# AshutoshNirkhe/KubernetesClusterCapacity

Hardware: AMD Instinct MI355X
Metric: node×spec fit evals/sec at 1M nodes × 4K specs; % of HBM roofline (higher is better)
Workload: dtype int64; 1 GPU; C4: 1000000 nodes x 20000000 pods x 4096 specs; reduce + fit prepare + fit + finalize; nodes=1000000, pods=20000000, containers_rank0=39602467, nodes_rank0=1000000, pods_rank0=19801877, pods_per_node=poisson, mean 20, specs=4096, parallelism=node-sharded x1

## Files before the change

### include/kcc.h

```cpp
#ifndef KCC_H
#define KCC_H

#include <stdint.h>

#ifdef __cplusplus
extern "C" {
#endif

#define KCC_ABI_VERSION 2

enum {
  KCC_OK = 0,
  KCC_EINVAL = -1,
  KCC_ENOMEM = -2,
  KCC_EHIP = -3,
  KCC_ENODEV = -4,
  KCC_ERCCL = -5,
  KCC_EFAULT = -6
};

enum {
  KCC_SPEC_OK = 0,
  KCC_SPEC_DIVZERO = 1,
  KCC_SPEC_FAULT = 2
// ... 93 lines not shown
int kcc_p2p_open(kcc_ctx* ctx, int rank, const uint8_t* handles );
int kcc_exchange_finalize_async(kcc_ctx* ctx, int64_t n_specs, const int64_t* d_partial,
                                int64_t* d_totals, int32_t* d_spec_err, void* stream);
int kcc_p2p_faults(kcc_ctx* ctx, int64_t* faults);

int kcc_profile_enable(kcc_ctx* ctx, int on);
int kcc_profile_read(kcc_ctx* ctx, double* reduce_ms, int64_t* reduce_launches, double* fit_ms,
                     int64_t* fit_launches);

int kcc_reduce_faults(kcc_ctx* ctx, int64_t* faults);
int kcc_clear_faults(kcc_ctx* ctx);

int kcc_set_fit_dense(kcc_ctx* ctx, int dense);
int kcc_set_clamp_in_fit(kcc_ctx* ctx, int mode);
int kcc_clamp_in_fit_used(kcc_ctx* ctx, int* used);
int kcc_fit_stream_rows(kcc_ctx* ctx, int64_t* streamed);

double kcc_last_slow_fraction(const kcc_ctx* ctx);

int kcc_fit_slow_pairs(kcc_ctx* ctx, int64_t* slow_pairs, int64_t* pairs);

enum {
  KCC_PARSE_OK = 1,
  KCC_PARSE_ERR = 0,
  KCC_PARSE_UNSUPPORTED = -1,
  KCC_PARSE_BADOFF = -2
};
int kcc_parse_cpu_millis(kcc_ctx* ctx, int64_t n, const char* bytes, int64_t n_bytes,
                         const int64_t* offsets, uint64_t* out, int8_t* status);
int kcc_parse_bytes(kcc_ctx* ctx, int64_t n, const char* bytes, int64_t n_bytes,
// ... 71 lines not shown
```

### kubernetesclustercapacity_amd/_lib.py

```python
from __future__ import annotations

import ctypes as C
import os
import re

_HERE = os.path.dirname(os.path.abspath(__file__))
LIB_PATH = os.path.join(_HERE, "libkcc.so")
HEADER_PATH = os.path.join(os.path.dirname(_HERE), "include", "kcc.h")

KCC_OK = 0
KCC_EINVAL = -1
KCC_ENOMEM = -2
KCC_EHIP = -3
KCC_ENODEV = -4
KCC_ERCCL = -5
KCC_EFAULT = -6
ERROR_NAMES = {
    KCC_EINVAL: "KCC_EINVAL", KCC_ENOMEM: "KCC_ENOMEM", KCC_EHIP: "KCC_EHIP",
    KCC_ENODEV: "KCC_ENODEV", KCC_ERCCL: "KCC_ERCCL", KCC_EFAULT: "KCC_EFAULT",
}
KCC_SPEC_OK = 0
KCC_SPEC_DIVZERO = 1
KCC_SPEC_FAULT = 2

# ... 12 lines not shown
    "kcc_reduce_requests_async": (_int, [_vp, _i64, _i64] + [_vp] * 10),
    "kcc_fit": (_int, [_vp, _i64] + [_vp] * 6 + [_i64] + [_vp] * 4),
    "kcc_capacity": (_int, [_vp, _i64, _i64] + [_vp] * 7 + [_i64] + [_vp] * 4),
    "kcc_fit_partial_async": (_int, [_vp, _i64] + [_vp] * 6 + [_i64] + [_vp] * 4),
    "kcc_fit_prepare_async": (_int, [_vp, _i64] + [_vp] * 6 + [_i64] + [_vp] * 4),
    "kcc_fit_run_async": (_int, [_vp, _i64, _i64, _vp, _vp]),
    "kcc_fit_finalize_async": (_int, [_vp, _i64, _vp, _vp, _vp, _vp]),
    "kcc_fit_async": (_int, [_vp, _i64] + [_vp] * 6 + [_i64] + [_vp] * 5),
    "kcc_capacity_partial_async": (_int, [_vp, _i64, _i64] + [_vp] * 10 + [_i64] + [_vp] * 3
                                   + [_int, _vp]),
    "kcc_capacity_async": (_int, [_vp, _i64, _i64] + [_vp] * 10 + [_i64] + [_vp] * 5),
    "kcc_set_node_shards": (_int, [_vp, _int]),
    "kcc_set_fit_dense": (_int, [_vp, _int]),
    "kcc_set_clamp_in_fit": (_int, [_vp, _int]),
    "kcc_clamp_in_fit_used": (_int, [_vp, C.POINTER(C.c_int)]),
    "kcc_fit_stream_rows": (_int, [_vp, C.POINTER(_i64)]),
    "kcc_reduce_faults": (_int, [_vp, C.POINTER(_i64)]),
    "kcc_clear_faults": (_int, [_vp]),
    "kcc_comm_unique_id": (_int, [_vp]),
    "kcc_comm_init": (_int, [_vp, _vp, _int, _int]),
    "kcc_allreduce_partial_async": (_int, [_vp, _i64, _vp, _vp]),
    "kcc_p2p_export": (_int, [_vp, _int, _i64, _vp]),
    "kcc_p2p_open": (_int, [_vp, _int, _vp]),
    "kcc_exchange_finalize_async": (_int, [_vp, _i64, _vp, _vp, _vp, _vp]),
    "kcc_p2p_faults": (_int, [_vp, C.POINTER(_i64)]),
    "kcc_profile_enable": (_int, [_vp, _int]),
    "kcc_profile_read": (_int, [_vp] + [C.POINTER(_dbl), C.POINTER(_i64)] * 2),
    "kcc_last_slow_fraction": (_dbl, [_vp]),
    "kcc_fit_slow_pairs": (_int, [_vp, C.POINTER(_i64), C.POINTER(_i64)]),
    "kcc_parse_cpu_millis": (_int, [_vp, _i64, _vp, _i64, _vp, _vp, _vp]),
# ... 61 lines not shown
```

### kubernetesclustercapacity_amd/csrc/kcc_abi.cpp

```cpp
#include "kcc.h"

#include <hip/hip_runtime.h>
#include <rccl/rccl.h>

#include <cstdio>
#include <cstdlib>
#include <cstring>
#include <string>
#include <vector>

#include "kcc_internal.h"

namespace {

struct DevBuf {
  void* p = nullptr;
  size_t bytes = 0;
};

hipError_t ensure(DevBuf& b, size_t bytes) {
  if (bytes == 0) bytes = 16;
  if (b.bytes >= bytes) return hipSuccess;
  if (b.p) (void)hipFree(b.p);
  b.p = nullptr;
// ... 38 lines not shown
  DevBuf fast_a, fast_b, slow, slow_list, srec, sperm, counters;
  DevBuf red_tail;
  DevBuf faults;
  DevBuf rank_arrive;
  DevBuf fit_q;
  bool fitq_dirty = true;
  DevBuf c_rank, c_bcnt, c_cs, c_ms, c_mrc, c_crm, c_dperm;
  DevBuf c_C, c_H2, c_H3, c_Crow, c_rec, c_dir;
  bool clamp_dirty = true;
  int64_t last_pairs = 0;
  int64_t c_stride = 0;
  int64_t h_stride = 0;
  int64_t d_stride = 0;
  bool fit_dense = false;
  int clamp_in_fit = -1;
  bool last_nc = false;
  DevBuf fast_cl;
  int stream_chunks = 0;
  int64_t prep_nodes = -1, prep_specs = -1;
  DevBuf ptr, cpu, mem, cpul, meml, used_cpu, used_mem, lim_cpu, lim_mem;
  DevBuf alloc_cpu, alloc_mem, alloc_pods, pod_count, spec_cpu, spec_mem, partial, totals, err;
  DevBuf p_bytes, p_off, p_out, p_st;
  DevBuf k_key;
  DevBuf g_group;
  DevBuf g_count, g_cursor, g_total, g_rec, g_rg, g_acc;
  DevBuf kb_counts, kb_tot, kb_sr, kb_sv;
  DevBuf kb_part, kb_arrive;
  DevBuf kb_esc_n, kb_esc_row, kb_esc_cpu, kb_esc_mem;
  DevBuf q_ptr, q_iptr, q_icpu, q_imem, q_rst, q_ocpu, q_omem, q_pcpu, q_pmem;
  DevBuf p2p_mbox, p2p_arrive;
// ... 428 lines not shown
  dv.stream_chunks = k;
  dv.prep_nodes = -1;
  dv.prep_specs = -1;
  hipStream_t rs = k > 1 ? dv.side : s;
  if (k > 1) {
    KCC_HIP(ctx, hipEventRecord(dv.ev_fork, s));
    KCC_HIP(ctx, hipStreamWaitEvent(dv.side, dv.ev_fork, 0));
  }
  const bool fuse_place = n_specs > 0;
  const bool fuse_rank = k == 1 && fuse_place && n_nodes > 0 && n_cont > 0;
  const bool nc = fuse_rank && n_specs <= kcc::CLAMP_LDS_SPECS && !dv.fit_dense &&
                  (dv.clamp_in_fit == 1 ||
                   (dv.clamp_in_fit < 0 && kcc::clamp_in_fit_auto(n_nodes, n_specs)));
  int32_t* const fast_cl = nc ? as<int32_t>(dv.fast_cl) : nullptr;
  dv.last_nc = nc;
  kcc::RankArgs ra = kcc::rank_args(n_specs, spec_cpu, spec_mem, clamp_of(dv),
                                    as<unsigned long long>(dv.counters),
                                    as<uint32_t>(dv.rank_arrive), nc);
  kcc::PlaceArgs pa = place_args(dv, n_specs, spec_cpu, spec_mem, partial);
  pa.no_ranks = nc ? 1 : 0;
  kcc::NpArgs np{};
  if (nc) {
    ra.done_flag = as<uint32_t>(dv.np_sync);
    np.n_place = (int32_t)((n_specs + 255) / 256);
    np.n_rows = (int32_t)((n_nodes + kcc::NP_ROWS_PER_WG - 1) / kcc::NP_ROWS_PER_WG);
    np.sync = as<uint32_t>(dv.np_sync);
    np.pa = pa;
    np.n = n_nodes;
    np.alloc_cpu = alloc_cpu;
    np.alloc_mem = alloc_mem;
// ... 48 lines not shown
    KCC_HIP(ctx, kcc::launch_node_prep(n, alloc_cpu + lo[c], alloc_mem + lo[c], alloc_pods + lo[c],
                                       pod_count + lo[c], used_cpu + lo[c], used_mem + lo[c],
                                       as<kcc::FitGroupA>(dv.fast_a) + lo[c] / kcc::FIT_GROUP,
                                       as<kcc::FitGroup>(dv.fast_b) + lo[c] / kcc::FIT_GROUP,
                                       as<kcc::SlowNode>(dv.slow) + lo[c],
                                       as<int64_t>(dv.slow_list) + lo[c], n_specs, clamp_of(dv),
                                       as<unsigned long long>(dv.counters),
                                       c, lo[c], n_nodes, s, dv.fit_dense,
                                       place_here ? &pa : nullptr));
    if (n == 0) continue;
    ProfPair pp{};
    if (dv.prof_on) {
      KCC_HIP(ctx, prof_event(dv, &pp.a));
      KCC_HIP(ctx, prof_event(dv, &pp.b));
    }
    KCC_HIP(ctx, kcc::launch_fit(n, as<kcc::FitGroupA>(dv.fast_a) + lo[c] / kcc::FIT_GROUP,
                                 as<kcc::FitGroup>(dv.fast_b) + lo[c] / kcc::FIT_GROUP,
                                 as<kcc::SlowNode>(dv.slow) + lo[c],
                                 as<int64_t>(dv.slow_list) + lo[c], n_specs, spec_prep_of(dv),
                                 partial, as<unsigned long long>(dv.counters),
                                 as<uint32_t>(dv.fit_q), c, n_nodes, s,
                                 as<const unsigned long long>(dv.faults), fast_cl,
                                 dv.prof_on ? pp.a : nullptr, dv.prof_on ? pp.b : nullptr));
    if (dv.prof_on) {
      pp.kind = 1;
      dv.prof_pending.push_back(pp);
    }
  }
  if (n_specs > 0 && nc) {
    dv.clamp_dirty = false;
    if (totals) return fit_finalize_dev(ctx, dv, n_specs, partial, totals, spec_err, s);
    return KCC_OK;
  }
  if (n_specs > 0) {
    if (n_nodes > 0)
      KCC_HIP(ctx, kcc::launch_clamp_apply(n_specs, n_nodes, clamp_of(dv),
                                           as<unsigned long long>(dv.counters), partial, s,
                                           fuse_fin ? &fin : nullptr));
    dv.clamp_dirty = false;
    if (totals && !fuse_fin)
      return fit_finalize_dev(ctx, dv, n_specs, partial, totals, spec_err, s);
  }
  return KCC_OK;
}
// ... 549 lines not shown

int kcc_clamp_in_fit_used(kcc_ctx* ctx, int* used) {
  if (!ctx || !used) return KCC_EINVAL;
  *used = 0;
  for (const Dev& dv : ctx->devs) *used |= dv.last_nc ? 1 : 0;
  return KCC_OK;
}

int kcc_set_clamp_in_fit(kcc_ctx* ctx, int mode) {
  if (!ctx) return KCC_EINVAL;
  if (mode < -1 || mode > 1) return fail(ctx, KCC_EINVAL, "mode: -1 (by size), 0 or 1");
  for (Dev& dv : ctx->devs) dv.clamp_in_fit = mode;
  return KCC_OK;
}

int kcc_fit_stream_rows(kcc_ctx* ctx, int64_t* streamed) {
  if (!ctx || !streamed) return ctx ? fail(ctx, KCC_EINVAL, "NULL output") : KCC_EINVAL;
  if (ctx->host_stream_rows >= 0) {
    *streamed = ctx->host_stream_rows;
    return KCC_OK;
  }
  Dev& dv = ctx->devs[0];
  KCC_HIP(ctx, hipSetDevice(dv.device));
  KCC_HIP(ctx, hipDeviceSynchronize());
  unsigned long long c[kcc::CNT_N] = {};
  if (dv.counters.p)
    KCC_HIP(ctx, hipMemcpy(c, dv.counters.p, sizeof(c), hipMemcpyDeviceToHost));
  int64_t t = 0;
  for (int k = 0; k < dv.stream_chunks && k < kcc::FIT_MAX_CHUNKS; ++k) t += (int64_t)c[kcc::CNT_STREAM + k];
  *streamed = t;
// ... 759 lines not shown
```

### kubernetesclustercapacity_amd/csrc/kcc_internal.h

```cpp
#pragma once
#include <hip/hip_runtime.h>
#include <stdint.h>

#if !defined(KCC_VARIANT_BUILD) &&                                                       \
    (defined(KCC_DIAG_RED_NOSTORE) || defined(KCC_DIAG_RED_LOADONLY) ||                  \
     defined(KCC_TIMELINE) || defined(KCC_DIAG_RED_GIVEUP) || defined(KCC_DIAG_P2P_GIVEUP) || \
     defined(KCC_DIAG_INLIB_COMM) || defined(KCC_DIAG_GA_NOATOM) ||                     \
     defined(KCC_DIAG_NP_NOSC1))
#error "a diagnostic KCC_* knob in a release build: use `make variant` (KCC_VARIANT_BUILD)"
#endif

namespace kcc {

struct RankArgs;
struct NpArgs;

constexpr int RED_PREFETCH = 1;
constexpr int RED_IPL = 8;
constexpr int RED_TILE = 64 * RED_IPL;
constexpr int RED_WAVES_PER_BLOCK = 4;
constexpr int64_t RED_MAX_NODES = (int64_t)1 << 28;
constexpr int RED_TAIL_WORDS = 8;
constexpr int RED_TAIL_TAG = 7;
constexpr uint64_t RED_TAG_READY = 1;
// ... 207 lines not shown
                            unsigned long long* counters, int chunk, int64_t row0,
                            int64_t call_nodes, hipStream_t s, bool dense = false,
                            const PlaceArgs* place = nullptr);
constexpr int64_t CLAMP_IN_FIT_PAIRS = 1100000000LL;
inline bool clamp_in_fit_auto(int64_t n_nodes, int64_t n_specs) {
  return n_specs <= CLAMP_LDS_SPECS && n_nodes * n_specs <= CLAMP_IN_FIT_PAIRS;
}

hipError_t launch_fit(int64_t n_nodes, const FitGroupA* fast_a, const FitGroup* fast_b,
                      const SlowNode* slow,
                      const int64_t* slow_list, int64_t n_specs, SpecPrep sp, int64_t* partial,
                      unsigned long long* counters, uint32_t* queue, int chunk,
                      int64_t grid_nodes, hipStream_t s, const unsigned long long* faults,
                      const int32_t* fast_cl = nullptr, hipEvent_t ev_start = nullptr,
                      hipEvent_t ev_stop = nullptr);
constexpr int64_t FIT_QSUBS_MAX = 32;
inline int64_t fit_queue_words(int64_t S) { return (S + 255) / 256 * FIT_QSUBS_MAX * 16; }

hipError_t launch_fit_finalize(int64_t n_specs, const int64_t* partial,
                               const int32_t* perm, int64_t* totals, int32_t* spec_err,
                               const unsigned long long* faults, hipStream_t s);
hipError_t launch_partial_add(int64_t n, int64_t* dst, const int64_t* src, hipStream_t s);

constexpr int P2P_MAX_RANKS = 8;
__host__ __device__ inline size_t p2p_flag_words(int W) { return (size_t)2 * W * 8; }
inline size_t p2p_mbox_bytes(int W, int64_t smax) {
  return 8 * (p2p_flag_words(W) + (size_t)2 * W * 2 * (size_t)smax);
}
struct P2PArgs {
  int64_t S, smax;
// ... 105 lines not shown
```

### kubernetesclustercapacity_amd/csrc/kcc_kernels.hip

```cpp

#include <hip/hip_ext.h>
#include <hip/hip_runtime.h>
#include <stdint.h>

#include <atomic>

#include "kcc_internal.h"

namespace kcc {

namespace {

#ifdef KCC_TIMELINE
__device__ uint64_t kcc_tl[8192][8];
#define KCC_TL(slot, k) \
  do { if (threadIdx.x == 0) kcc_tl[(slot)][(k)] = __builtin_amdgcn_s_memrealtime(); } while (0)
#define KCC_TLV(slot, k, v) \
  do { if (threadIdx.x == 0) kcc_tl[(slot)][(k)] = (v); } while (0)
#else
#define KCC_TL(slot, k) do { } while (0)
#define KCC_TLV(slot, k, v) do { } while (0)
#endif

typedef __attribute__((address_space(3))) unsigned long long lds_ull;
// ... 1449 lines not shown
  rec.rc = normal ? recip_up_f64(c) : 0.0;
  rec.rm = normal ? recip_up_f64((uint64_t)m) : 0.0;
  rec.rcf = cls == SPEC_A ? recip_up_f32(c) : 0.0f;
  rec.cls = cls;
  rec.pad = 0;
  sp.rec[pos] = rec;
  sp.perm[pos] = (int32_t)i;
  partial[i] = 0;
  partial[S + i] = device_faulted(pa.faults) ? (int64_t)SPEC_FAULT_MARK : 0;
  if (!normal || pa.no_ranks) return;
  cw.dperm[x] = (int32_t)pos;
}


constexpr int CP_THREADS = 1024;
constexpr int CP_WAVES = CP_THREADS / 64;
constexpr int64_t C_FULL_CELLS = 4624;
constexpr int H_CELLS = 65 * 64;
__host__ __device__ inline bool clamp_c_full(int64_t T) { return (T + 2) * (T + 2) <= C_FULL_CELLS; }

constexpr int CP_PW = 4096;
constexpr int64_t CP_SPLIT = 4;
constexpr int CP_RB = 8;
__device__ __forceinline__ void clamp_consume_bin(const ClampWork& cw, int64_t bin, uint64_t* tab,
                                                  uint32_t* w_lo, uint32_t* w_off, uint64_t* scratch,
                                                  uint32_t h, uint32_t G) {
  constexpr int PPT = CP_PW / CP_THREADS;
  const int tid = threadIdx.x, lane = tid & 63, wv = tid >> 6;
  uint32_t* wsum = reinterpret_cast<uint32_t*>(scratch);
  for (int64_t p0 = 0; p0 < cw.n_pass; p0 += CP_PW) {
    const int np = (int)(cw.n_pass - p0 < CP_PW ? cw.n_pass - p0 : CP_PW);
    uint32_t lo[PPT], cnt[PPT];
#pragma unroll
    for (int u = 0; u < PPT; ++u) {
      const int p = tid * PPT + u;
      lo[u] = 0;
      cnt[u] = 0;
      if (p < np) {
        const uint32_t* d = cw.dir + (p0 + p) * cw.d_stride + bin;
        lo[u] = d[0];
        cnt[u] = d[1];
      }
    }
    uint32_t ts = 0;
#pragma unroll
    for (int u = 0; u < PPT; ++u) {
      cnt[u] -= lo[u];
      ts += cnt[u];
    }
    uint32_t inc = ts;
#pragma unroll
    for (int d = 1; d < 64; d <<= 1) {
      const uint32_t t = __shfl_up(inc, d, 64);
      if (lane >= d) inc += t;
    }
    if (lane == 63) wsum[wv] = inc;
    __syncthreads();
    uint32_t before = 0, total = 0;
#pragma unroll
    for (int w2 = 0; w2 < CP_WAVES; ++w2) {
      const uint32_t t = wsum[w2];
      before += w2 < wv ? t : 0u;
      total += t;
    }
    uint32_t run = before + inc - ts;
#pragma unroll
    for (int u = 0; u < PPT; ++u) {
      const int p = tid * PPT + u;
      w_lo[p] = lo[u];
      w_off[p] = run;
      run += cnt[u];
    }
    if (tid == 0) w_off[CP_PW] = total;
    __syncthreads();
    int top = 1;
    while (2 * top <= np) top *= 2;
    auto search = [&](uint32_t j) {
      int p = 0;
      for (int st = top; st >= 1; st >>= 1)
        if (w_off[p + st] <= j) p += st;
      return p;
    };
    const uint32_t s0 = (uint32_t)((uint64_t)total * h / G), s1 = (uint32_t)((uint64_t)total * (h + 1) / G);
    const uint32_t per_w = (s1 - s0 + CP_WAVES * 64 - 1) / (CP_WAVES * 64) * 64;
    const uint32_t J0 = s0 + (uint32_t)wv * per_w;
    const uint32_t J1 = J0 + per_w < s1 ? J0 + per_w : s1;
    int p = J0 + lane < J1 ? search(J0 + lane) : 0;
    uint32_t nxt = w_off[p + 1], gb = w_lo[p] - w_off[p];
    const uint64_t* rec0 = cw.rec + p0 * cw.pass_recs;
    auto load_batch = [&](uint64_t (&rv)[CP_RB], uint32_t jb) {
#pragma unroll
      for (int u = 0; u < CP_RB; ++u) {
        const uint32_t j = jb + (uint32_t)(64 * u + lane);
        rv[u] = 0;
        if (j < J1) {
          if (j >= nxt) {
            p = w_off[p + 2] <= j ? search(j) : p + 1;
            nxt = w_off[p + 1];
            gb = w_lo[p] - w_off[p];
          }
          rv[u] = rec0[(int64_t)p * cw.pass_recs + (uint32_t)(j + gb)];
        }
      }
    };
    auto add_batch = [&](const uint64_t (&rv)[CP_RB], uint32_t jb) {
#pragma unroll
      for (int u = 0; u < CP_RB; ++u)
        if (jb + (uint32_t)(64 * u + lane) < J1)
          atomicAdd(reinterpret_cast<unsigned long long*>(&tab[(uint32_t)rv[u]]),
                    (unsigned long long)(int64_t)(int32_t)(rv[u] >> 32));
    };
    const uint32_t step = 64u * CP_RB;
    uint64_t ra[CP_RB], rb[CP_RB];
    load_batch(ra, J0);
    for (uint32_t jb = J0; jb < J1; jb += 2 * step) {
      load_batch(rb, jb + step);
      add_batch(ra, jb);
      load_batch(ra, jb + 2 * step);
      add_batch(rb, jb + step);
    }
    __syncthreads();
  }
}

__device__ __forceinline__ void clamp_apply_bin(const ClampWork& cw, int64_t S,
                                                int64_t* __restrict__ partial, int64_t nN,
                                                int64_t u, uint32_t G, uint32_t h) {
  __shared__ uint64_t tab[H_CELLS];
  __shared__ uint64_t ctot[CP_WAVES][64];
  __shared__ uint64_t colsum[128];
  __shared__ uint32_t pos_s[64];
  __shared__ uint32_t cp_lo[CP_PW];
  __shared__ uint32_t cp_off[CP_PW + 1];
  const int64_t T = (nN + 63) / 64, W = T + 2;
  KCC_TL(1024 + blockIdx.x % 1024, 0);
  const int tid = threadIdx.x, lane = tid & 63, wv = tid >> 6;
  const bool x_side = u < T;
  const int64_t g = x_side ? u : u - T;
  const bool full = clamp_c_full(T);
  const int64_t q = 64 * g + lane;
  uint32_t other = 0xffffffffu;
  if (wv == 0 || wv == CP_WAVES - 1) other = (x_side ? cw.mr_c : cw.cr_m)[q];
  if (tid < 128) colsum[tid] = 0;
  const bool binned = clamp_binned(S);
  int64_t* H = (x_side ? cw.H2 : cw.H3) + g * H_CELLS;
  constexpr int PER = (H_CELLS + CP_THREADS - 1) / CP_THREADS;
  uint64_t v[PER];
#pragma unroll
  for (int k = 0; k < PER; ++k) {
    const int e = tid + CP_THREADS * k;
    v[k] = 0;
    if (!binned) {
#pragma unroll
      for (int c = 0; c < H2_COPIES; ++c) v[k] += e < H_CELLS ? (uint64_t)H[c * cw.h_stride + e] : 0ull;
    }
  }
  constexpr int CPER = (int)((C_FULL_CELLS + CP_THREADS - 1) / CP_THREADS);
  uint64_t cv[CPER];
  const int64_t c0 = (g + 1) * W, c1 = W * W;
  const bool do_c = x_side && full && h == 0;
#pragma unroll
  for (int k = 0; k < CPER; ++k) {
    const int64_t e = c0 + tid + CP_THREADS * k;
    cv[k] = 0;
    if (do_c && e < c1) {
#pragma unroll
      for (int c = 0; c < C_COPIES; ++c) cv[k] += (uint64_t)cw.C[c * cw.c_stride + e];
    }
  }
#pragma unroll
  for (int k = 0; k < PER; ++k) {
    const int e = tid + CP_THREADS * k;
    if (e < H_CELLS) {
      tab[e] = v[k];
      if (!binned) {
#pragma unroll
        for (int c = 0; c < H2_COPIES; ++c) H[c * cw.h_stride + e] = 0;
      }
    }
  }
  __syncthreads();
  KCC_TL(1024 + blockIdx.x % 1024, 1);
  if (binned) clamp_consume_bin(cw, x_side ? g : T + g, tab, cp_lo, cp_off, &ctot[0][0], h, G);
  KCC_TL(1024 + blockIdx.x % 1024, 2);
  if (do_c) {
#pragma unroll
    for (int k = 0; k < CPER; ++k) {
      const int64_t e = c0 + tid + CP_THREADS * k;
      if (e < c1 && cv[k]) atomicAdd(reinterpret_cast<unsigned long long*>(&colsum[e % W]), cv[k]);
    }
  }
  int32_t p = 0x7fffffff;
  if (wv == 0 && q < nN) p = cw.dperm[x_side ? q : (int64_t)other];
  for (int k = wv; k < 65; k += CP_WAVES) {
    const uint64_t sr = wave_incl_scan_u64(tab[k * 64 + 63 - lane]);
    tab[k * 64 + 63 - lane] = sr;
  }
  if (wv == CP_WAVES - 1) {
    uint32_t pos = 0;
    for (int l = 0; l < 64; ++l) pos += (uint32_t)__builtin_amdgcn_readlane((int)other, l) < other ? 1u : 0u;
    pos_s[lane] = pos;
  }
  __syncthreads();
  constexpr int KCH = (65 + CP_WAVES - 1) / CP_WAVES;
  const int k0 = wv * KCH, k1 = k0 + KCH < 65 ? k0 + KCH : 65;
  {
    const uint32_t posl = pos_s[lane];
    uint64_t part = 0;
    for (int k = k0; k < k1; ++k)
      part += (lane < 63 && (uint32_t)k > posl) ? tab[k * 64 + lane + 1] : 0ull;
    ctot[wv][lane] = part;
  }
  __syncthreads();
  if (wv != 0) return;
  KCC_TL(1024 + blockIdx.x % 1024, 3);
  uint64_t csuf = 0;
  if (do_c) {
    uint64_t carry = 0;
    for (int ch = 1; ch >= 0; --ch) {
      const int col = ch * 64 + 63 - lane;
      uint64_t sv = col < W ? colsum[col] : 0ull;
      sv = wave_incl_scan_u64(sv) + carry;
      carry = readlane_u64(sv, 63);
      if (col < W) colsum[col] = sv;
    }
    const uint32_t gy1 = other == 0xffffffffu ? 0xffffffffu : (other >> 6) + 1;
    csuf = gy1 < W ? colsum[gy1] : 0ull;
  }
  if (q >= nN) return;
  uint64_t d = csuf;
#pragma unroll
  for (int w2 = 0; w2 < CP_WAVES; ++w2) d += ctot[w2][lane];
  if (x_side && !full && h == 0) {
    const int64_t gy = other >> 6;
    uint64_t part[8] = {};
    for (int64_t G = g + 1; G <= T + 1; G += 8) {
#pragma unroll
      for (int r = 0; r < 8; ++r)
        part[r] += G + r <= T + 1 ? (uint64_t)cw.Crow[(G + r) * W + gy + 1] : 0ull;
    }
#pragma unroll
    for (int r = 0; r < 8; ++r) d += part[r];
  }
  if (d && p < clamp_n_pure(nN, S)) atomic_add_u64(reinterpret_cast<uint64_t*>(&partial[p]), 0ull - d);
  KCC_TL(1024 + blockIdx.x % 1024, 4);
}

__device__ void fused_finalize(const FinArgs& fin, int64_t S, const int64_t* partial,
// ... 28 lines not shown
      fin.totals[dst[k]] = e[k] != 0 || fk ? 0 : t[k];
      fin.spec_err[dst[k]] = fk ? SPEC_ERR_FAULT : e[k] != 0 ? SPEC_ERR_DIV0 : 0;
    }
  }
}

__global__ __launch_bounds__(CP_THREADS) void clamp_apply_kernel(ClampWork cw,
                                                                 const unsigned long long* __restrict__ counters,
                                                                 int64_t S, int64_t* __restrict__ partial,
                                                                 FinArgs fin) {
  const int64_t nN = clamp_n_normal(counters);
  const int64_t T = (nN + 63) / 64;
  const int64_t Tm = (S + 63) / 64;
  const uint32_t G = gridDim.x / (uint32_t)(2 * Tm), h = blockIdx.x / (uint32_t)(2 * Tm);
  const int64_t u = blockIdx.x % (uint32_t)(2 * Tm);
  if (u < 2 * T) clamp_apply_bin(cw, S, partial, nN, u, G, h);
  if (fin.totals) fused_finalize(fin, S, partial, fin.arrive, gridDim.x, 0, S);
}

__global__ __launch_bounds__(256) void clamp_crows_kernel(ClampWork cw,
                                                          const unsigned long long* __restrict__ counters) {
  const int64_t nN = clamp_n_normal(counters);
  const int64_t T = (nN + 63) / 64, W = T + 2;
  const int64_t G = (int64_t)blockIdx.x * 4 + (threadIdx.x >> 6);
  const int lane = threadIdx.x & 63;
  if (nN == 0 || clamp_c_full(T) || G >= W) return;
  uint64_t carry = 0;
  for (int64_t ch = (W + 63) / 64 - 1; ch >= 0; --ch) {
    const int64_t gy = ch * 64 + 63 - lane;
    uint64_t v = 0;
#pragma unroll
// ... 350 lines not shown
  }
  KCC_TL(2048 + b % 4096, 3);
}

template <bool CL>
__global__ __launch_bounds__(256) KCC_FIT_ATTR void fit_kernel(
    int64_t n_nodes, uint32_t* __restrict__ queue, const FitGroupA* __restrict__ fast_a,
    const FitGroup* __restrict__ fast_b, const SlowNode* __restrict__ slow,
    const int64_t* __restrict__ slow_list, int64_t S, const SpecRec* __restrict__ specs,
    int64_t* __restrict__ partial, unsigned long long* __restrict__ counters, int32_t chunk,
    int32_t gx, int32_t gy, const int32_t* __restrict__ fast_cl,
    const unsigned long long* __restrict__ faults) {
  __shared__ uint32_t q_slot[2];
  fit_body<CL>(n_nodes, queue, fast_a, fast_b, slow, slow_list, S, specs, partial, counters, chunk,
               gx, gy, fast_cl, faults, (int32_t)blockIdx.x, q_slot);
}

__global__ void fit_finalize_kernel(int64_t S, const int64_t* __restrict__ partial,
                                    const int32_t* __restrict__ perm, int64_t* __restrict__ totals,
                                    int32_t* __restrict__ spec_err,
                                    const unsigned long long* __restrict__ faults) {
  const int64_t i = (int64_t)blockIdx.x * blockDim.x + threadIdx.x;
  if (i >= S) return;
  const int32_t dst = perm[i];
  const bool err = partial[S + i] != 0;
  const bool faulted = device_faulted(faults) || (uint64_t)partial[S + i] >= SPEC_FAULT_MARK;
  totals[dst] = err || faulted ? 0 : partial[i];
  spec_err[dst] = faulted ? SPEC_ERR_FAULT : err ? SPEC_ERR_DIV0 : 0;
}

// ... 311 lines not shown
  const int64_t gy = fit_grid_y(n_nodes, n_specs, grid_nodes);
  const int64_t blocks = gx * ((gy + 7) / 8 * 8);
  if (blocks > 0x7fffffffLL || gy > 0x7fffffffLL) return hipErrorInvalidValue;
  auto kern = fast_cl ? fit_kernel<true> : fit_kernel<false>;
  if (ev_start || ev_stop)
    hipExtLaunchKernelGGL(kern, dim3((unsigned)blocks), dim3(256), 0, s, ev_start, ev_stop, 0, n_nodes,
                          queue, fast_a, fast_b, slow, slow_list, n_specs, sp.rec, partial, counters,
                          (int32_t)chunk, (int32_t)gx, (int32_t)gy, fast_cl, faults);
  else
    hipLaunchKernelGGL(kern, dim3((unsigned)blocks), dim3(256), 0, s, n_nodes, queue, fast_a,
                       fast_b, slow, slow_list, n_specs, sp.rec, partial, counters, (int32_t)chunk,
                       (int32_t)gx, (int32_t)gy, fast_cl, faults);
  return hipGetLastError();
}

hipError_t launch_fit_finalize(int64_t n_specs, const int64_t* partial, const int32_t* perm,
                               int64_t* totals, int32_t* spec_err,
                               const unsigned long long* faults, hipStream_t s) {
  if (n_specs <= 0) return hipSuccess;
  hipLaunchKernelGGL(fit_finalize_kernel, dim3(grid_for(n_specs, 256, 1 << 30)), dim3(256), 0, s,
                     n_specs, partial, perm, totals, spec_err, faults);
  return hipGetLastError();
}

hipError_t launch_exchange_finalize(const P2PArgs& a, hipStream_t s) {
  if (a.S <= 0) return hipSuccess;
  if (a.S > a.smax || a.W < 1 || a.W > P2P_MAX_RANKS || a.rank < 0 || a.rank >= a.W ||
      !a.epoch || !a.faults || !a.arrive)
    return hipErrorInvalidValue;
  hipLaunchKernelGGL(exchange_finalize_kernel, dim3(grid_for(a.S, 256, P2P_MAX_WG)), dim3(256), 0, s, a);
// ... 22 lines not shown
```

### kubernetesclustercapacity_amd/engine.py

```python
from __future__ import annotations

import ctypes as C
from dataclasses import dataclass

import numpy as np

from . import _lib

COMM_ID_BYTES = 128
P2P_HANDLE_BYTES = 64


class KccError(RuntimeError):
    def __init__(self, code: int, msg: str):
        super().__init__(f"{_lib.ERROR_NAMES.get(code, code)}: {msg}")
        self.code = code


def _arr(x, dtype) -> np.ndarray:
    a = np.ascontiguousarray(x, dtype=dtype)
    return a


def _p(a) -> C.c_void_p | None:
# ... 400 lines not shown
        self._check(self._lib.kcc_profile_read(self._h, C.byref(rm), C.byref(rn), C.byref(fm),
                                               C.byref(fn)))
        return rm.value, rn.value, fm.value, fn.value

    def set_fit_dense(self, dense: bool):
        self._check(self._lib.kcc_set_fit_dense(self._h, 1 if dense else 0))

    def set_clamp_in_fit(self, mode: int):
        self._check(self._lib.kcc_set_clamp_in_fit(self._h, int(mode)))

    def clamp_in_fit_used(self) -> bool:
        v = C.c_int()
        self._check(self._lib.kcc_clamp_in_fit_used(self._h, C.byref(v)))
        return bool(v.value)

    def fit_stream_rows(self) -> int:
        v = C.c_int64()
        self._check(self._lib.kcc_fit_stream_rows(self._h, C.byref(v)))
        return v.value

    def reduce_faults(self) -> int:
        v = C.c_int64()
        self._check(self._lib.kcc_reduce_faults(self._h, C.byref(v)))
        return v.value

    def clear_faults(self):
        self._check(self._lib.kcc_clear_faults(self._h))

    def fit_slow_pairs(self):
        a, b = C.c_int64(), C.c_int64()
# ... 38 lines not shown
```

Measured before the change: 14670 billion evals/s.

## Run clamp histogram apply inside fit kernel as side workgroups

```diff
diff --git a/include/kcc.h b/include/kcc.h
--- a/include/kcc.h
+++ b/include/kcc.h
@@ -131,6 +131,8 @@
 int kcc_set_fit_dense(kcc_ctx* ctx, int dense);
 int kcc_set_clamp_in_fit(kcc_ctx* ctx, int mode);
 int kcc_clamp_in_fit_used(kcc_ctx* ctx, int* used);
+int kcc_set_clamp_ride(kcc_ctx* ctx, int mode);
+int kcc_clamp_ride_used(kcc_ctx* ctx, int* used);
 int kcc_fit_stream_rows(kcc_ctx* ctx, int64_t* streamed);
 
 double kcc_last_slow_fraction(const kcc_ctx* ctx);
diff --git a/kubernetesclustercapacity_amd/_lib.py b/kubernetesclustercapacity_amd/_lib.py
--- a/kubernetesclustercapacity_amd/_lib.py
+++ b/kubernetesclustercapacity_amd/_lib.py
@@ -50,6 +50,8 @@
     "kcc_set_fit_dense": (_int, [_vp, _int]),
     "kcc_set_clamp_in_fit": (_int, [_vp, _int]),
     "kcc_clamp_in_fit_used": (_int, [_vp, C.POINTER(C.c_int)]),
+    "kcc_set_clamp_ride": (_int, [_vp, _int]),
+    "kcc_clamp_ride_used": (_int, [_vp, C.POINTER(C.c_int)]),
     "kcc_fit_stream_rows": (_int, [_vp, C.POINTER(_i64)]),
     "kcc_reduce_faults": (_int, [_vp, C.POINTER(_i64)]),
     "kcc_clear_faults": (_int, [_vp]),
diff --git a/kubernetesclustercapacity_amd/csrc/kcc_abi.cpp b/kubernetesclustercapacity_amd/csrc/kcc_abi.cpp
--- a/kubernetesclustercapacity_amd/csrc/kcc_abi.cpp
+++ b/kubernetesclustercapacity_amd/csrc/kcc_abi.cpp
@@ -76,6 +76,8 @@
   int64_t d_stride = 0;
   bool fit_dense = false;
   int clamp_in_fit = -1;
+  int clamp_ride = -1;
+  bool last_ride = false;
   bool last_nc = false;
   DevBuf fast_cl;
   int stream_chunks = 0;
@@ -534,6 +536,10 @@
                    (dv.clamp_in_fit < 0 && kcc::clamp_in_fit_auto(n_nodes, n_specs)));
   int32_t* const fast_cl = nc ? as<int32_t>(dv.fast_cl) : nullptr;
   dv.last_nc = nc;
+  const bool ride = k == 1 && !nc && n_nodes > 0 && n_specs > 0 && n_specs <= kcc::CLAMP_LDS_SPECS &&
+                    (dv.clamp_ride >= 1 ||
+                     (dv.clamp_ride < 0 && kcc::clamp_ride_auto(n_nodes, n_specs)));
+  dv.last_ride = ride;
   kcc::RankArgs ra = kcc::rank_args(n_specs, spec_cpu, spec_mem, clamp_of(dv),
                                     as<unsigned long long>(dv.counters),
                                     as<uint32_t>(dv.rank_arrive), nc);
@@ -612,6 +618,15 @@
       KCC_HIP(ctx, prof_event(dv, &pp.a));
       KCC_HIP(ctx, prof_event(dv, &pp.b));
     }
+    if (ride)
+      KCC_HIP(ctx, kcc::launch_fit_clamp(n, as<kcc::FitGroupA>(dv.fast_a), as<kcc::FitGroup>(dv.fast_b),
+                                         as<kcc::SlowNode>(dv.slow), as<int64_t>(dv.slow_list),
+                                         n_specs, spec_prep_of(dv), partial,
+                                         as<unsigned long long>(dv.counters),
+                                         as<uint32_t>(dv.fit_q), clamp_of(dv), s,
+                                         as<const unsigned long long>(dv.faults),
+                                         dv.prof_on ? pp.a : nullptr, dv.prof_on ? pp.b : nullptr));
+    else
     KCC_HIP(ctx, kcc::launch_fit(n, as<kcc::FitGroupA>(dv.fast_a) + lo[c] / kcc::FIT_GROUP,
                                  as<kcc::FitGroup>(dv.fast_b) + lo[c] / kcc::FIT_GROUP,
                                  as<kcc::SlowNode>(dv.slow) + lo[c],
@@ -625,7 +640,7 @@
       dv.prof_pending.push_back(pp);
     }
   }
-  if (n_specs > 0 && nc) {
+  if (n_specs > 0 && (nc || ride)) {
     dv.clamp_dirty = false;
     if (totals) return fit_finalize_dev(ctx, dv, n_specs, partial, totals, spec_err, s);
     return KCC_OK;
@@ -1205,6 +1220,20 @@
   return KCC_OK;
 }
 
+int kcc_clamp_ride_used(kcc_ctx* ctx, int* used) {
+  if (!ctx || !used) return KCC_EINVAL;
+  *used = 0;
+  for (const Dev& dv : ctx->devs) *used |= dv.last_ride ? 1 : 0;
+  return KCC_OK;
+}
+
+int kcc_set_clamp_ride(kcc_ctx* ctx, int mode) {
+  if (!ctx) return KCC_EINVAL;
+  if (mode < -1 || mode > 1) return fail(ctx, KCC_EINVAL, "mode: -1 (by size), 0 or 1");
+  for (Dev& dv : ctx->devs) dv.clamp_ride = mode;
+  return KCC_OK;
+}
+
 int kcc_fit_stream_rows(kcc_ctx* ctx, int64_t* streamed) {
   if (!ctx || !streamed) return ctx ? fail(ctx, KCC_EINVAL, "NULL output") : KCC_EINVAL;
   if (ctx->host_stream_rows >= 0) {
diff --git a/kubernetesclustercapacity_amd/csrc/kcc_internal.h b/kubernetesclustercapacity_amd/csrc/kcc_internal.h
--- a/kubernetesclustercapacity_amd/csrc/kcc_internal.h
+++ b/kubernetesclustercapacity_amd/csrc/kcc_internal.h
@@ -245,6 +245,17 @@
                       int64_t grid_nodes, hipStream_t s, const unsigned long long* faults,
                       const int32_t* fast_cl = nullptr, hipEvent_t ev_start = nullptr,
                       hipEvent_t ev_stop = nullptr);
+hipError_t launch_fit_clamp(int64_t n_nodes, const FitGroupA* fast_a, const FitGroup* fast_b,
+                            const SlowNode* slow, const int64_t* slow_list, int64_t n_specs,
+                            SpecPrep sp, int64_t* partial, unsigned long long* counters,
+                            uint32_t* queue, ClampWork cw, hipStream_t s,
+                            const unsigned long long* faults, hipEvent_t ev_start = nullptr,
+                            hipEvent_t ev_stop = nullptr);
+int64_t fit_clamp_side_blocks(int64_t n_specs, int32_t* parts = nullptr);
+inline bool clamp_ride_auto(int64_t n_nodes, int64_t n_specs) {
+  return n_specs <= CLAMP_LDS_SPECS && n_nodes * n_specs > CLAMP_IN_FIT_PAIRS;
+}
+
 constexpr int64_t FIT_QSUBS_MAX = 32;
 inline int64_t fit_queue_words(int64_t S) { return (S + 255) / 256 * FIT_QSUBS_MAX * 16; }
 
diff --git a/kubernetesclustercapacity_amd/csrc/kcc_kernels.hip b/kubernetesclustercapacity_amd/csrc/kcc_kernels.hip
--- a/kubernetesclustercapacity_amd/csrc/kcc_kernels.hip
+++ b/kubernetesclustercapacity_amd/csrc/kcc_kernels.hip
@@ -1487,7 +1487,6 @@
 
 
 constexpr int CP_THREADS = 1024;
-constexpr int CP_WAVES = CP_THREADS / 64;
 constexpr int64_t C_FULL_CELLS = 4624;
 constexpr int H_CELLS = 65 * 64;
 __host__ __device__ inline bool clamp_c_full(int64_t T) { return (T + 2) * (T + 2) <= C_FULL_CELLS; }
@@ -1495,14 +1494,33 @@
 constexpr int CP_PW = 4096;
 constexpr int64_t CP_SPLIT = 4;
 constexpr int CP_RB = 8;
+constexpr int CP_SIDE_THREADS = 256;
+constexpr int CP_SIDE_SLICES = 4;
+constexpr int CP_SIDE_PW = 256;
+constexpr int CP_SIDE_RB = 4;
+constexpr int64_t CP_SIDE_SPLIT = 32;
+constexpr int64_t CP_SIDE_PER_CU = 4;
+template <int NT, int NSL>
+struct ClampShape {
+  static_assert(NT % 64 == 0 && 64 % NSL == 0, "whole waves, equal slices after the first");
+  static constexpr int NW = NT / 64;
+  static constexpr int PW = NSL == 1 ? CP_PW : CP_SIDE_PW;
+  static constexpr int RB = NSL == 1 ? CP_RB : CP_SIDE_RB;
+  static constexpr int REST = 64 / NSL;
+  static constexpr int FIRST = 65 - (NSL - 1) * REST;
+  static_assert(PW % NT == 0, "whole passes per thread");
+};
+template <int NT, int NSL>
 __device__ __forceinline__ void clamp_consume_bin(const ClampWork& cw, int64_t bin, uint64_t* tab,
                                                   uint32_t* w_lo, uint32_t* w_off, uint64_t* scratch,
-                                                  uint32_t h, uint32_t G) {
-  constexpr int PPT = CP_PW / CP_THREADS;
+                                                  uint32_t h, uint32_t G, uint32_t c_lo, uint32_t c_n) {
+  using SH = ClampShape<NT, NSL>;
+  constexpr int PW = SH::PW, RB = SH::RB, NW = SH::NW;
+  constexpr int PPT = PW / NT;
   const int tid = threadIdx.x, lane = tid & 63, wv = tid >> 6;
   uint32_t* wsum = reinterpret_cast<uint32_t*>(scratch);
-  for (int64_t p0 = 0; p0 < cw.n_pass; p0 += CP_PW) {
-    const int np = (int)(cw.n_pass - p0 < CP_PW ? cw.n_pass - p0 : CP_PW);
+  for (int64_t p0 = 0; p0 < cw.n_pass; p0 += PW) {
+    const int np = (int)(cw.n_pass - p0 < PW ? cw.n_pass - p0 : PW);
     uint32_t lo[PPT], cnt[PPT];
 #pragma unroll
     for (int u = 0; u < PPT; ++u) {
@@ -1531,7 +1549,7 @@
     __syncthreads();
     uint32_t before = 0, total = 0;
 #pragma unroll
-    for (int w2 = 0; w2 < CP_WAVES; ++w2) {
+    for (int w2 = 0; w2 < NW; ++w2) {
       const uint32_t t = wsum[w2];
       before += w2 < wv ? t : 0u;
       total += t;
@@ -1544,7 +1562,7 @@
       w_off[p] = run;
       run += cnt[u];
     }
-    if (tid == 0) w_off[CP_PW] = total;
+    if (tid == 0) w_off[PW] = total;
     __syncthreads();
     int top = 1;
     while (2 * top <= np) top *= 2;
@@ -1555,15 +1573,15 @@
       return p;
     };
     const uint32_t s0 = (uint32_t)((uint64_t)total * h / G), s1 = (uint32_t)((uint64_t)total * (h + 1) / G);
-    const uint32_t per_w = (s1 - s0 + CP_WAVES * 64 - 1) / (CP_WAVES * 64) * 64;
+    const uint32_t per_w = (s1 - s0 + NW * 64 - 1) / (NW * 64) * 64;
     const uint32_t J0 = s0 + (uint32_t)wv * per_w;
     const uint32_t J1 = J0 + per_w < s1 ? J0 + per_w : s1;
     int p = J0 + lane < J1 ? search(J0 + lane) : 0;
     uint32_t nxt = w_off[p + 1], gb = w_lo[p] - w_off[p];
     const uint64_t* rec0 = cw.rec + p0 * cw.pass_recs;
-    auto load_batch = [&](uint64_t (&rv)[CP_RB], uint32_t jb) {
-#pragma unroll
-      for (int u = 0; u < CP_RB; ++u) {
+    auto load_batch = [&](uint64_t (&rv)[RB], uint32_t jb) {
+#pragma unroll
+      for (int u = 0; u < RB; ++u) {
         const uint32_t j = jb + (uint32_t)(64 * u + lane);
         rv[u] = 0;
         if (j < J1) {
@@ -1576,15 +1594,23 @@
         }
       }
     };
-    auto add_batch = [&](const uint64_t (&rv)[CP_RB], uint32_t jb) {
-#pragma unroll
-      for (int u = 0; u < CP_RB; ++u)
-        if (jb + (uint32_t)(64 * u + lane) < J1)
-          atomicAdd(reinterpret_cast<unsigned long long*>(&tab[(uint32_t)rv[u]]),
-                    (unsigned long long)(int64_t)(int32_t)(rv[u] >> 32));
+    auto add_batch = [&](const uint64_t (&rv)[RB], uint32_t jb) {
+#pragma unroll
+      for (int u = 0; u < RB; ++u)
+        if (jb + (uint32_t)(64 * u + lane) < J1) {
+          if constexpr (NSL == 1) {
+            atomicAdd(reinterpret_cast<unsigned long long*>(&tab[(uint32_t)rv[u]]),
+                      (unsigned long long)(int64_t)(int32_t)(rv[u] >> 32));
+          } else {
+            const uint32_t cell = (uint32_t)rv[u] - c_lo;
+            if (cell < c_n)
+              atomicAdd(reinterpret_cast<unsigned long long*>(&tab[cell]),
+                        (unsigned long long)(int64_t)(int32_t)(rv[u] >> 32));
+          }
+        }
     };
-    const uint32_t step = 64u * CP_RB;
-    uint64_t ra[CP_RB], rb[CP_RB];
+    const uint32_t step = 64u * RB;
+    uint64_t ra[RB], rb[RB];
     load_batch(ra, J0);
     for (uint32_t jb = J0; jb < J1; jb += 2 * step) {
       load_batch(rb, jb + step);
@@ -1596,15 +1622,18 @@
   }
 }
 
+template <int NT, int NSL>
 __device__ __forceinline__ void clamp_apply_bin(const ClampWork& cw, int64_t S,
                                                 int64_t* __restrict__ partial, int64_t nN,
-                                                int64_t u, uint32_t G, uint32_t h) {
-  __shared__ uint64_t tab[H_CELLS];
-  __shared__ uint64_t ctot[CP_WAVES][64];
+                                                int64_t u, uint32_t G, uint32_t h, int sl = 0) {
+  using SH = ClampShape<NT, NSL>;
+  constexpr int NW = SH::NW, PW = SH::PW;
+  __shared__ uint64_t tab[SH::FIRST * 64];
+  __shared__ uint64_t ctot[NW][64];
   __shared__ uint64_t colsum[128];
   __shared__ uint32_t pos_s[64];
-  __shared__ uint32_t cp_lo[CP_PW];
-  __shared__ uint32_t cp_off[CP_PW + 1];
+  __shared__ uint32_t cp_lo[PW];
+  __shared__ uint32_t cp_off[PW + 1];
   const int64_t T = (nN + 63) / 64, W = T + 2;
   KCC_TL(1024 + blockIdx.x % 1024, 0);
   const int tid = threadIdx.x, lane = tid & 63, wv = tid >> 6;
@@ -1613,76 +1642,99 @@
   const bool full = clamp_c_full(T);
   const int64_t q = 64 * g + lane;
   uint32_t other = 0xffffffffu;
-  if (wv == 0 || wv == CP_WAVES - 1) other = (x_side ? cw.mr_c : cw.cr_m)[q];
+  if (wv == 0 || wv == NW - 1) other = (x_side ? cw.mr_c : cw.cr_m)[q];
   if (tid < 128) colsum[tid] = 0;
-  const bool binned = clamp_binned(S);
+  const bool binned = NSL > 1 || clamp_binned(S);
   int64_t* H = (x_side ? cw.H2 : cw.H3) + g * H_CELLS;
-  constexpr int PER = (H_CELLS + CP_THREADS - 1) / CP_THREADS;
-  uint64_t v[PER];
-#pragma unroll
-  for (int k = 0; k < PER; ++k) {
-    const int e = tid + CP_THREADS * k;
-    v[k] = 0;
-    if (!binned) {
-#pragma unroll
-      for (int c = 0; c < H2_COPIES; ++c) v[k] += e < H_CELLS ? (uint64_t)H[c * cw.h_stride + e] : 0ull;
-    }
-  }
-  constexpr int CPER = (int)((C_FULL_CELLS + CP_THREADS - 1) / CP_THREADS);
-  uint64_t cv[CPER];
+  constexpr int PER = NSL == 1 ? (H_CELLS + NT - 1) / NT : 1;
+  [[maybe_unused]] uint64_t v[PER];
+  if constexpr (NSL == 1) {
+#pragma unroll
+    for (int k = 0; k < PER; ++k) {
+      const int e = tid + NT * k;
+      v[k] = 0;
+      if (!binned) {
+#pragma unroll
+        for (int c = 0; c < H2_COPIES; ++c) v[k] += e < H_CELLS ? (uint64_t)H[c * cw.h_stride + e] : 0ull;
+      }
+    }
+  }
+  constexpr int CPER = (int)((C_FULL_CELLS + NT - 1) / NT);
+  [[maybe_unused]] uint64_t cv[NSL == 1 ? CPER : 1];
   const int64_t c0 = (g + 1) * W, c1 = W * W;
-  const bool do_c = x_side && full && h == 0;
-#pragma unroll
-  for (int k = 0; k < CPER; ++k) {
-    const int64_t e = c0 + tid + CP_THREADS * k;
-    cv[k] = 0;
-    if (do_c && e < c1) {
-#pragma unroll
-      for (int c = 0; c < C_COPIES; ++c) cv[k] += (uint64_t)cw.C[c * cw.c_stride + e];
-    }
-  }
-#pragma unroll
-  for (int k = 0; k < PER; ++k) {
-    const int e = tid + CP_THREADS * k;
-    if (e < H_CELLS) {
-      tab[e] = v[k];
-      if (!binned) {
-#pragma unroll
-        for (int c = 0; c < H2_COPIES; ++c) H[c * cw.h_stride + e] = 0;
-      }
-    }
-  }
-  __syncthreads();
+  const bool do_c = x_side && full && h == 0 && sl == 0;
+  if constexpr (NSL == 1) {
+#pragma unroll
+    for (int k = 0; k < CPER; ++k) {
+      const int64_t e = c0 + tid + NT * k;
+      cv[k] = 0;
+      if (do_c && e < c1) {
+#pragma unroll
+        for (int c = 0; c < C_COPIES; ++c) cv[k] += (uint64_t)cw.C[c * cw.c_stride + e];
+      }
+    }
+#pragma unroll
+    for (int k = 0; k < PER; ++k) {
+      const int e = tid + NT * k;
+      if (e < H_CELLS) {
+        tab[e] = v[k];
+        if (!binned) {
+#pragma unroll
+          for (int c = 0; c < H2_COPIES; ++c) H[c * cw.h_stride + e] = 0;
+        }
+      }
+    }
+    __syncthreads();
+  }
+  const int kb = sl ? SH::FIRST + (sl - 1) * SH::REST : 0;
+  const int kn = sl ? SH::REST : SH::FIRST;
+  if constexpr (NSL > 1) {
+    for (int e = tid; e < kn * 64; e += NT) tab[e] = 0;
+    __syncthreads();
+  }
   KCC_TL(1024 + blockIdx.x % 1024, 1);
-  if (binned) clamp_consume_bin(cw, x_side ? g : T + g, tab, cp_lo, cp_off, &ctot[0][0], h, G);
+  if (binned)
+    clamp_consume_bin<NT, NSL>(cw, x_side ? g : T + g, tab, cp_lo, cp_off, &ctot[0][0], h, G,
+                               (uint32_t)kb * 64u, (uint32_t)kn * 64u);
   KCC_TL(1024 + blockIdx.x % 1024, 2);
-  if (do_c) {
-#pragma unroll
-    for (int k = 0; k < CPER; ++k) {
-      const int64_t e = c0 + tid + CP_THREADS * k;
-      if (e < c1 && cv[k]) atomicAdd(reinterpret_cast<unsigned long long*>(&colsum[e % W]), cv[k]);
+  if constexpr (NSL == 1) {
+    if (do_c) {
+#pragma unroll
+      for (int k = 0; k < CPER; ++k) {
+        const int64_t e = c0 + tid + NT * k;
+        if (e < c1 && cv[k]) atomicAdd(reinterpret_cast<unsigned long long*>(&colsum[e % W]), cv[k]);
+      }
     }
   }
   int32_t p = 0x7fffffff;
   if (wv == 0 && q < nN) p = cw.dperm[x_side ? q : (int64_t)other];
-  for (int k = wv; k < 65; k += CP_WAVES) {
+  for (int k = wv; k < kn; k += NW) {
     const uint64_t sr = wave_incl_scan_u64(tab[k * 64 + 63 - lane]);
     tab[k * 64 + 63 - lane] = sr;
   }
-  if (wv == CP_WAVES - 1) {
+  if (wv == NW - 1) {
     uint32_t pos = 0;
     for (int l = 0; l < 64; ++l) pos += (uint32_t)__builtin_amdgcn_readlane((int)other, l) < other ? 1u : 0u;
     pos_s[lane] = pos;
   }
   __syncthreads();
-  constexpr int KCH = (65 + CP_WAVES - 1) / CP_WAVES;
-  const int k0 = wv * KCH, k1 = k0 + KCH < 65 ? k0 + KCH : 65;
+  const int kch = (kn + NW - 1) / NW;
+  const int k0 = wv * kch, k1 = k0 + kch < kn ? k0 + kch : kn;
   {
     const uint32_t posl = pos_s[lane];
     uint64_t part = 0;
     for (int k = k0; k < k1; ++k)
-      part += (lane < 63 && (uint32_t)k > posl) ? tab[k * 64 + lane + 1] : 0ull;
+      part += (lane < 63 && (uint32_t)(kb + k) > posl) ? tab[k * 64 + lane + 1] : 0ull;
     ctot[wv][lane] = part;
+  }
+  if constexpr (NSL > 1) {
+    if (do_c)
+      for (int64_t e = c0 + tid; e < c1; e += NT) {
+        uint64_t cs = 0;
+#pragma unroll
+        for (int c = 0; c < C_COPIES; ++c) cs += (uint64_t)cw.C[c * cw.c_stride + e];
+        if (cs) atomicAdd(reinterpret_cast<unsigned long long*>(&colsum[e % W]), cs);
+      }
   }
   __syncthreads();
   if (wv != 0) return;
@@ -1703,8 +1755,8 @@
   if (q >= nN) return;
   uint64_t d = csuf;
 #pragma unroll
-  for (int w2 = 0; w2 < CP_WAVES; ++w2) d += ctot[w2][lane];
-  if (x_side && !full && h == 0) {
+  for (int w2 = 0; w2 < NW; ++w2) d += ctot[w2][lane];
+  if (x_side && !full && h == 0 && sl == 0) {
     const int64_t gy = other >> 6;
     uint64_t part[8] = {};
     for (int64_t G = g + 1; G <= T + 1; G += 8) {
@@ -1763,7 +1815,7 @@
   const int64_t Tm = (S + 63) / 64;
   const uint32_t G = gridDim.x / (uint32_t)(2 * Tm), h = blockIdx.x / (uint32_t)(2 * Tm);
   const int64_t u = blockIdx.x % (uint32_t)(2 * Tm);
-  if (u < 2 * T) clamp_apply_bin(cw, S, partial, nN, u, G, h);
+  if (u < 2 * T) clamp_apply_bin<CP_THREADS, 1>(cw, S, partial, nN, u, G, h);
   if (fin.totals) fused_finalize(fin, S, partial, fin.arrive, gridDim.x, 0, S);
 }
 
@@ -2144,6 +2196,30 @@
   __shared__ uint32_t q_slot[2];
   fit_body<CL>(n_nodes, queue, fast_a, fast_b, slow, slow_list, S, specs, partial, counters, chunk,
                gx, gy, fast_cl, faults, (int32_t)blockIdx.x, q_slot);
+}
+
+__global__ __launch_bounds__(256) KCC_FIT_ATTR void fit_clamp_kernel(
+    int64_t n_nodes, uint32_t* __restrict__ queue, const FitGroupA* __restrict__ fast_a,
+    const FitGroup* __restrict__ fast_b, const SlowNode* __restrict__ slow,
+    const int64_t* __restrict__ slow_list, int64_t S, const SpecRec* __restrict__ specs,
+    int64_t* __restrict__ partial, unsigned long long* __restrict__ counters, int32_t gx,
+    int32_t gy, const unsigned long long* __restrict__ faults, ClampWork cw, int32_t n_side,
+    int32_t side_g) {
+  static_assert(CP_SIDE_THREADS == 256, "the clamp role runs in the fit's workgroups");
+  __shared__ uint32_t q_slot[2];
+  if ((int32_t)blockIdx.x < n_side) {
+    const int64_t nN = clamp_n_normal(counters);
+    const int64_t T = (nN + 63) / 64;
+    const uint32_t Tm2 = 2u * (uint32_t)((S + 63) / 64);
+    const uint32_t t = blockIdx.x / Tm2, u = blockIdx.x % Tm2;
+    const uint32_t h = t % (uint32_t)side_g, sl = t / (uint32_t)side_g;
+    if (sl < (uint32_t)CP_SIDE_SLICES && u < 2 * T)
+      clamp_apply_bin<CP_SIDE_THREADS, CP_SIDE_SLICES>(cw, S, partial, nN, u, (uint32_t)side_g, h,
+                                                       (int)sl);
+    return;
+  }
+  fit_body<false>(n_nodes, queue, fast_a, fast_b, slow, slow_list, S, specs, partial, counters, 0,
+                  gx, gy, nullptr, faults, (int32_t)blockIdx.x - n_side, q_slot);
 }
 
 __global__ void fit_finalize_kernel(int64_t S, const int64_t* __restrict__ partial,
@@ -2485,6 +2561,45 @@
   return hipGetLastError();
 }
 
+int64_t fit_clamp_side_blocks(int64_t n_specs, int32_t* parts) {
+  const int64_t Tm = (n_specs + 63) / 64;
+  int dev = 0, cus = 0;
+  if (hipGetDevice(&dev) != hipSuccess ||
+      hipDeviceGetAttribute(&cus, hipDeviceAttributeMultiprocessorCount, dev) != hipSuccess || cus < 1)
+    cus = 256;
+  int64_t G = 1;
+  while (G < CP_SIDE_SPLIT && 2 * Tm * CP_SIDE_SLICES * G * 2 <= (int64_t)cus * CP_SIDE_PER_CU) G *= 2;
+  if (parts) *parts = (int32_t)G;
+  return (2 * Tm * CP_SIDE_SLICES * G + 7) / 8 * 8;
+}
+
+hipError_t launch_fit_clamp(int64_t n_nodes, const FitGroupA* fast_a, const FitGroup* fast_b,
+                            const SlowNode* slow, const int64_t* slow_list, int64_t n_specs,
+                            SpecPrep sp, int64_t* partial, unsigned long long* counters,
+                            uint32_t* queue, ClampWork cw, hipStream_t s,
+                            const unsigned long long* faults, hipEvent_t ev_start,
+                            hipEvent_t ev_stop) {
+  if (n_nodes <= 0 || n_specs <= 0 || n_specs > CLAMP_LDS_SPECS) return hipErrorInvalidValue;
+  cw.n_pass = clamp_passes(n_nodes);
+  cw.pass_recs = 2 * clamp_pass_rows(n_nodes);
+  int32_t parts = 1;
+  const int64_t n_side = fit_clamp_side_blocks(n_specs, &parts);
+  const int64_t gx = (n_specs + FIT_SPW - 1) / FIT_SPW;
+  const int64_t gy = fit_grid_y(n_nodes, n_specs, n_nodes);
+  const int64_t blocks = n_side + gx * ((gy + 7) / 8 * 8);
+  if (blocks > 0x7fffffffLL || gy > 0x7fffffffLL) return hipErrorInvalidValue;
+  if (ev_start || ev_stop)
+    hipExtLaunchKernelGGL(fit_clamp_kernel, dim3((unsigned)blocks), dim3(256), 0, s, ev_start,
+                          ev_stop, 0, n_nodes, queue, fast_a, fast_b, slow, slow_list, n_specs,
+                          sp.rec, partial, counters, (int32_t)gx, (int32_t)gy, faults, cw,
+                          (int32_t)n_side, parts);
+  else
+    hipLaunchKernelGGL(fit_clamp_kernel, dim3((unsigned)blocks), dim3(256), 0, s, n_nodes, queue,
+                       fast_a, fast_b, slow, slow_list, n_specs, sp.rec, partial, counters,
+                       (int32_t)gx, (int32_t)gy, faults, cw, (int32_t)n_side, parts);
+  return hipGetLastError();
+}
+
 hipError_t launch_fit_finalize(int64_t n_specs, const int64_t* partial, const int32_t* perm,
                                int64_t* totals, int32_t* spec_err,
                                const unsigned long long* faults, hipStream_t s) {
diff --git a/kubernetesclustercapacity_amd/engine.py b/kubernetesclustercapacity_amd/engine.py
--- a/kubernetesclustercapacity_amd/engine.py
+++ b/kubernetesclustercapacity_amd/engine.py
@@ -438,6 +438,14 @@
         self._check(self._lib.kcc_clamp_in_fit_used(self._h, C.byref(v)))
         return bool(v.value)
 
+    def set_clamp_ride(self, mode: int):
+        self._check(self._lib.kcc_set_clamp_ride(self._h, int(mode)))
+
+    def clamp_ride_used(self) -> bool:
+        v = C.c_int()
+        self._check(self._lib.kcc_clamp_ride_used(self._h, C.byref(v)))
+        return bool(v.value)
+
     def fit_stream_rows(self) -> int:
         v = C.c_int64()
         self._check(self._lib.kcc_fit_stream_rows(self._h, C.byref(v)))
```

Measured after the change: 14970 billion evals/s (median of 6 runs). 2.1% higher.
